# datavizweb/async-rl-tensorflow

Measured on NVIDIA B200. Metric: env_frames_per_sec, higher is better.
Workload: dtype f32

## Files before the change

async-rl-tensorflow_b200/csrc/api.cu:

```cuda
#include <stdarg.h>
#include <stdlib.h>
#include <string.h>

#include "common.cuh"

namespace arl {

static thread_local char g_err[512] = "";

void set_error(const char* fmt, ...) {
  va_list ap;
  va_start(ap, fmt);
  vsnprintf(g_err, sizeof(g_err), fmt, ap);
  va_end(ap);
}

int cuda_fail(cudaError_t e, const char* what) {
  set_error("CUDA error %d (%s) at %s", (int)e, cudaGetErrorString(e), what);
  return ARL_ERR_CUDA;
}

static long long g_launches = 0;
void count_launch() { __atomic_fetch_add(&g_launches, 1, __ATOMIC_RELAXED); }

static int g_num_sms[64] = {0};
int num_sms() {
  int dev = 0;
  if (cudaGetDevice(&dev) != cudaSuccess) dev = 0;
  const int n = g_num_sms[dev & 63];
  return n > 0 ? n : 148;
}

int preprocess_init(int device);
int conv_init();
int heads_init();

}

using namespace arl;

extern "C" const char* arl_last_error(void) { return g_err; }
extern "C" int arl_version(void) { return 100; }
extern "C" int64_t arl_launch_count(int reset) {
  const long long v = __atomic_load_n(&g_launches, __ATOMIC_RELAXED);
  if (reset) __atomic_store_n(&g_launches, 0, __ATOMIC_RELAXED);
  return (int64_t)v;
}

extern "C" int arl_init(int device) {
  int count = 0;
  ARL_CUDA(cudaGetDeviceCount(&count));
  ARL_REQUIRE(device >= 0 && device < count, "arl_init: device %d not in [0,%d)", device, count);
  int prev = 0;
  ARL_CUDA(cudaGetDevice(&prev));
  ARL_CUDA(cudaSetDevice(device));
  cudaDeviceProp prop;
  ARL_CUDA(cudaGetDeviceProperties(&prop, device));
  if (prop.major != 10) {
    set_error("arl_init: device %d is sm_%d%d; this library is built for sm_100a (B200) only",
              device, prop.major, prop.minor);
    cudaSetDevice(prev);
    return ARL_ERR_UNSUPPORTED;
  }
  g_num_sms[device & 63] = prop.multiProcessorCount;
  int rc = preprocess_init(device);
  if (rc == ARL_OK) rc = conv_init();
  if (rc == ARL_OK) rc = heads_init();
  cudaSetDevice(prev);
  return rc;
}

extern "C" int arl_param_layout(int action_size, int64_t* offsets) {
  ARL_REQUIRE(offsets, "arl_param_layout: null pointer");
  ARL_REQUIRE(action_size >= 1 && action_size <= ARL_MAX_ACTIONS,
              "arl_param_layout: action_size %d outside [1,%d]", action_size, ARL_MAX_ACTIONS);
  const ParamLayout L = param_layout(action_size);
  memcpy(offsets, L.off, sizeof(L.off));
  return ARL_OK;
}

extern "C" int64_t arl_backward_workspace_bytes(int action_size) {
  (void)action_size;
  return (int64_t)8 * ARL_A2_ELEMS * ARL_FC * sizeof(float) + (1 << 20);
}

extern "C" int64_t arl_a2_block_rows(int num_envs) {
  if (num_envs <= 16384) return num_envs;
  for (int c = 16384; c >= 2048; c -= 128)
    if (num_envs % c == 0) return c;
  return num_envs;
}

static int forward_step(const float* params, float* prepared, int action_size, const uint8_t* ring,
                        int num_envs, int ring_slots, int first_slot, float* a1, float* a2, float* h,
                        float* logits, float* probs, float* value, int32_t* actions, int64_t env_id_base,
                        int64_t step, const int64_t* step_dev, uint64_t seed, void* stream) {
  const int chunk = (int)arl_a2_block_rows(num_envs);
  for (int off = 0; off < num_envs; off += chunk) {
    const int n = num_envs - off < chunk ? num_envs - off : chunk;
    float* a1c = a1 + (size_t)off * 3200;
    float* a2c = a2 + (size_t)off * ARL_A2_ELEMS;
    float* hc = h + (size_t)off * ARL_FC;
    int rc = arl_conv1_forward(prepared, ring + (size_t)off * ring_slots * kPlane, a1c, n, ring_slots,
                               first_slot, 1, stream);
    if (rc) return rc;
    rc = arl_conv2_forward(prepared, a1c, a2c, n, stream);
    if (rc) return rc;
    rc = arl_fc_heads_forward(params, prepared, action_size, a2c, hc, logits + (size_t)off * action_size,
                              probs + (size_t)off * action_size, value + off,
                              actions ? actions + off : nullptr, env_id_base + off, step, step_dev, seed, n,
                              stream);
    if (rc) return rc;
  }
  return ARL_OK;
}

extern "C" int arl_forward(const float* params, float* prepared, int refresh_prepared, int action_size,
                           const uint8_t* ring, int num_envs, int ring_slots, int first_slot, int steps,
                           float* a1, float* a2, float* h, float* logits, float* probs, float* value,
                           void* stream) {
  const int64_t N = (int64_t)num_envs * steps;
  int rc = ARL_OK;
  if (refresh_prepared) rc = arl_prepare_weights(params, prepared, stream);
  if (rc) return rc;
  if (steps == 1)
    return forward_step(params, prepared, action_size, ring, num_envs, ring_slots, first_slot, a1, a2, h,
                        logits, probs, value, nullptr, 0, 0, nullptr, 0, stream);
  rc = arl_conv1_forward(prepared, ring, a1, num_envs, ring_slots, first_slot, steps, stream);
  if (rc) return rc;
  rc = arl_conv2_forward(prepared, a1, a2, N, stream);
  if (rc) return rc;
  return arl_fc_heads_forward(params, prepared, action_size, a2, h, logits, probs, value, nullptr, 0, 0,
                              nullptr, 0, N, stream);
}

extern "C" int arl_forward_sample(const float* params, float* prepared, int refresh_prepared, int action_size,
                                  const uint8_t* ring, int num_envs, int ring_slots, int first_slot,
                                  float* a1, float* a2, float* h, float* logits, float* probs, float* value,
                                  int32_t* actions, int64_t env_id_base, int64_t step,
                                  const int64_t* step_dev, uint64_t seed, void* stream) {
  ARL_REQUIRE(actions, "arl_forward_sample: null pointer");
  int rc = ARL_OK;
  if (refresh_prepared) rc = arl_prepare_weights(params, prepared, stream);
  if (rc) return rc;
  return forward_step(params, prepared, action_size, ring, num_envs, ring_slots, first_slot, a1, a2, h,
                      logits, probs, value, actions, env_id_base, step, step_dev, seed, stream);
}

extern "C" int arl_backward(const float* params, const float* prepared, int action_size,
                            const uint8_t* ring, int num_envs, int ring_slots, int first_slot,
                            int steps, const float* a1,
                            const float* a2, const float* h, const float* dlogits,
                            const float* dvalue, float* d_h, float* d_a2, float* d_a1, float* grads,
                            void* workspace, float tensor_scale, int allreduce, void* stream) {
  ARL_REQUIRE(tensor_scale > 0.f, "arl_backward: tensor_scale must be > 0");
  const int64_t N = (int64_t)num_envs * steps;
  const float unscale = 1.0f / tensor_scale;
  int rc = arl_heads_backward(params, action_size, h, dlogits, dvalue, d_h, grads, workspace, N,
                              tensor_scale, stream);
  if (rc) return rc;
  rc = arl_fc_backward(prepared, a2, arl_a2_block_rows(num_envs), d_h, d_a2, grads, workspace, N, unscale, stream);
  if (rc) return rc;
  const bool comm = allreduce && arl_comm_size() > 1;
  const ParamLayout L = param_layout(action_size);
  static const bool overlap = [] { const char* e = getenv("ARL_ALLREDUCE_OVERLAP"); return e && e[0] == '1'; }();
  if (comm && !overlap) {
    rc = arl_conv2_backward(prepared, a1, d_a2, d_a1, grads, workspace, N, unscale, stream);
    if (rc) return rc;
    rc = arl_conv1_backward(ring, d_a1, grads, workspace, num_envs, ring_slots, first_slot, steps, unscale, stream);
    if (rc) return rc;
    return arl_allreduce_grads(grads, L.off[ARL_NUM_TENSORS], stream);
  }
  if (comm) {
    rc = arl_allreduce_begin(grads, L.off[T_L4W], L.off[ARL_NUM_TENSORS] - L.off[T_L4W], stream);
    if (rc) return rc;
  }
  rc = arl_conv2_backward(prepared, a1, d_a2, d_a1, grads, workspace, N, unscale, stream);
  if (rc) return rc;
  rc = arl_conv1_backward(ring, d_a1, grads, workspace, num_envs, ring_slots, first_slot, steps,
                          unscale, stream);
  if (rc || !comm) return rc;
  rc = arl_allreduce_begin(grads, 0, L.off[T_L4W], stream);
  if (rc) return rc;
// ... 3 lines not shown
```

async-rl-tensorflow_b200/csrc/convs_tc.cu:

```cuda
#include <stdlib.h>

#include "gemm_tc.cuh"

namespace arl {

int reduce_partials(const float* partials, float* out, int num_partials, int n, cudaStream_t stream);
int reduce_partials_scaled(const float* partials, float* out, int num_partials, int n, float alpha,
                           cudaStream_t stream);

namespace {
using tc::TileCoord;
using tc::kTileM;

__device__ __forceinline__ void load8(const float* p, float (&x)[8]) {
  const float4 x0 = __ldg(reinterpret_cast<const float4*>(p));
  const float4 x1 = __ldg(reinterpret_cast<const float4*>(p) + 1);
  x[0] = x0.x; x[1] = x0.y; x[2] = x0.z; x[3] = x0.w;
  x[4] = x1.x; x[5] = x1.y; x[6] = x1.z; x[7] = x1.w;
}
__device__ __forceinline__ TileCoord row_tile(int item) {
  TileCoord t;
  t.mt = item; t.nt = 0; t.ks = 0; t.k_begin = 0; t.k_end = 0;
  return t;
}
// ... 174 lines not shown
  int num_samples;
};
struct Conv1Fwd : tc::PolicyBase {
  using Args = Conv1FwdArgs;
  static constexpr int GW = 21, GROWS = 441, TROWS = 150;
  static constexpr int PL = (TROWS + 1) * 16;
  static constexpr int EPI_SETS = 2, PROD_WARPS = 8, STAGES = 8, STAGE_BYTES = 4 * PL;
  static constexpr int PLB = 49 * 16, B_IMG = 16 * PLB, SCALE_OFF = B_IMG, BIAS_OFF = B_IMG + 16;
  static constexpr int RES_BYTES = B_IMG + 16 + 64;
  static constexpr int ACC_COLS = 64, OUT_COLS = 16, LO_DELTA = 16, SEG = 16;
  static constexpr bool CUSTOM_EPI = true, ACC_LIMBS3 = true;
  static __device__ __forceinline__ int acc_col(int c) { return c; }
  static __device__ __forceinline__ int num_items(const Args& g) { return (int)((g.rows + 127) / 128); }
  static __device__ __forceinline__ TileCoord coord(const Args&, int item) { return row_tile(item); }
  static __device__ __forceinline__ int num_stages(const Args&, const TileCoord&) { return 1; }
  static __device__ __forceinline__ void load_resident(const Args& g, uint8_t* res, int ptid, int nthr) {
    copy_image<RES_BYTES>(res, g.w_img, ptid, nthr);
  }
  static __device__ __forceinline__ void build_image(const float* params, uint8_t* res, int ptid, int nthr) {
    struct { const float* params; } g{params};
    uint32_t* smax = reinterpret_cast<uint32_t*>(res + SCALE_OFF + 12);
    if (ptid == 0) *smax = 0u;
    asm volatile("bar.sync 1, %0;" ::"r"(nthr) : "memory");
    float m = 0.f;
    for (int i = ptid; i < 4096; i += nthr) m = fmaxf(m, fabsf(g.params[i]));
#pragma unroll
    for (int o = 16; o > 0; o >>= 1) m = fmaxf(m, __shfl_xor_sync(0xffffffffu, m, o));
    if ((ptid & 31) == 0) atomicMax(smax, __float_as_uint(m));
    asm volatile("bar.sync 1, %0;" ::"r"(nthr) : "memory");
    const float s = fmaxf(__uint_as_float(*smax), 1e-30f), inv = 1.0f / s;
    if (ptid == 0) {
      float* sc = reinterpret_cast<float*>(res + SCALE_OFF);
      sc[0] = s * (1.0f / 64.0f); sc[1] = s * (1.0f / 8192.0f); sc[2] = s * (1.0f / 1048576.0f);
    }
    for (int ch = ptid; ch < 16 * 16; ch += nthr) {
      const int co = ch & 15, kc = ch >> 4, tap = kc >> 2, c = kc & 3, a = tap >> 1, b = tap & 1;
      uint32_t l0[4] = {0, 0, 0, 0}, l1[4] = {0, 0, 0, 0}, l2[4] = {0, 0, 0, 0};
#pragma unroll
      for (int e = 0; e < 16; ++e) {
        const int i = e >> 2, j = e & 3;
        const float v = g.params[(((4 * a + i) * 8 + 4 * b + j) * 4 + c) * 16 + co] * inv * 64.0f;
        const float r0 = rintf(v), f1 = (v - r0) * 128.0f, r1 = rintf(f1), r2 = rintf((f1 - r1) * 128.0f);
        l0[e >> 2] |= ((uint32_t)(int)r0 & 0xFFu) << (8 * (e & 3));
        l1[e >> 2] |= ((uint32_t)(int)r1 & 0xFFu) << (8 * (e & 3));
        l2[e >> 2] |= ((uint32_t)(int)r2 & 0xFFu) << (8 * (e & 3));
      }
      uint8_t* d = res + kc * PLB + co * 16;
      *reinterpret_cast<uint4*>(d) = make_uint4(l0[0], l0[1], l0[2], l0[3]);
      *reinterpret_cast<uint4*>(d + 16 * 16) = make_uint4(l1[0], l1[1], l1[2], l1[3]);
      *reinterpret_cast<uint4*>(d + 32 * 16) = make_uint4(l2[0], l2[1], l2[2], l2[3]);
    }
    if (ptid < 16) reinterpret_cast<float*>(res + BIAS_OFF)[ptid] = g.params[4096 + ptid];
  }
  static __device__ __forceinline__ void load_stage(const Args& g, const TileCoord& t, int,
                                                    uint8_t* st, int glane, int gsize, Prod&) {
    const int64_t valid = (int64_t)g.num_samples * GROWS - (int64_t)t.mt * 128;
    if (valid >= TROWS) return;
    for (int c = glane; c < TROWS * 4; c += gsize) {
      const int r = c % TROWS, kc = c / TROWS;
      if (r >= valid) *reinterpret_cast<uint4*>(st + kc * PL + r * 16) = make_uint4(0u, 0u, 0u, 0u);
    }
  }
  static __device__ __forceinline__ bool bulk_stage(const Args& g, const TileCoord& t, int, uint8_t* st,
                                                    int glane, int, uint64_t* full) {
    if (glane >= 8) return false;
    const int sgm = glane >> 2, c = glane & 3;
    const int xr0 = t.mt * 128;
    const int n0 = xr0 / GROWS, q0 = xr0 - n0 * GROWS;
    const int first = min(GROWS - q0, TROWS);
    const int n = n0 + sgm;
    int cnt = sgm == 0 ? first : TROWS - first;
    if (n >= g.num_samples) cnt = 0;
    mbar_expect_tx(full, (uint32_t)cnt * 16u);
    if (cnt > 0) {
      const int tt = n / g.geo.num_envs, b = n - tt * g.geo.num_envs;
      const int slot = (g.geo.first_slot + tt + c) % g.geo.ring_slots;
      const uint8_t* src = g.geo.ring + ((size_t)b * g.geo.ring_slots + slot) * kPlane + (sgm == 0 ? q0 : 0) * 16;
      bulk_g2s(st + c * PL + (sgm == 0 ? 0 : first) * 16, src, (uint32_t)cnt * 16u, full);
    }
    return true;
  }
  static __device__ __forceinline__ void issue(const Args&, const TileCoord&, int, uint32_t st,
                                               uint32_t res, uint32_t d) {
    constexpr uint32_t idesc = tc::make_idesc_i8(48);
    const uint64_t da0 = tc::make_sdesc(st, PL), db0 = tc::make_sdesc(res, PLB);
#pragma unroll
    for (int tap = 0; tap < 4; ++tap) {
#pragma unroll
      for (int k32 = 0; k32 < 2; ++k32) {
        const uint64_t da = tc::sdesc_advance(da0, ((tap >> 1) * GW + (tap & 1)) * 16 + 2 * k32 * PL);
        const uint64_t db = tc::sdesc_advance(db0, (tap * 4 + 2 * k32) * PLB);
        tc::umma_i8(d, da, db, idesc, (tap | k32) != 0 ? 1u : 0u);
      }
    }
  }
  static __device__ __forceinline__ void custom_epilogue(const Args& g, const TileCoord& t,
                                                         const uint8_t* res, uint32_t taddr, int row,
                                                         EpiPre&, EpiState&) {
    const float* sc = reinterpret_cast<const float*>(res + SCALE_OFF);
    float v[16];
    {
      float a[8], b[8];
      tc::tmem_ld8_limbs3(taddr, taddr + 16, taddr + 32, sc[0], sc[1], sc[2], a);
      tc::tmem_ld8_limbs3(taddr + 8, taddr + 24, taddr + 40, sc[0], sc[1], sc[2], b);
#pragma unroll
      for (int e = 0; e < 8; ++e) { v[e] = a[e]; v[8 + e] = b[e]; }
    }
    const int xr = t.mt * 128 + row, n = xr / GROWS;
    const int q = xr - n * GROWS, y = q / GW, x = q - y * GW;
    if (n >= g.num_samples || y >= 20 || x >= 20) return;
    const float2* bias = reinterpret_cast<const float2*>(res + BIAS_OFF);
    uint32_t h[8];
#pragma unroll
    for (int e = 0; e < 8; ++e) {
      const float2 bb = bias[e];
      const float o0 = fmaxf(fmaf(v[2 * e], 1.0f / 255.0f, bb.x), 0.f);
      const float o1 = fmaxf(fmaf(v[2 * e + 1], 1.0f / 255.0f, bb.y), 0.f);
      h[e] = tc::pack_h2(o0, o1);
    }
    uint8_t* d = g.a1s + (size_t)n * kA1sSample + a1s_offset(y, x, 0);
    *reinterpret_cast<uint4*>(d) = make_uint4(h[0], h[1], h[2], h[3]);
    *reinterpret_cast<uint4*>(d + kA1sPlane) = make_uint4(h[4], h[5], h[6], h[7]);
  }
};

struct Conv2FwdArgs {
  const uint8_t* w_img;
  const uint8_t* a1s;
  uint8_t* a2s;
  int64_t rows;
  int num_samples;
  int reverse;
};
struct Conv2Fwd : tc::PolicyBase {
  using Args = Conv2FwdArgs;
  static constexpr int GW = 10, GROWS = 100, TROWS = 140;
  static constexpr int PL = (TROWS + 1) * 16, IMG = 8 * PL;
  static constexpr int EPI_SETS = 2, PROD_WARPS = 6, STAGES = 6, STAGE_BYTES = IMG;
  static constexpr int PLB = 65 * 16, B_IMG = 32 * PLB, BIAS_OFF = B_IMG, RES_BYTES = B_IMG + 128;
  static constexpr int ACC_COLS = 64, OUT_COLS = 32, LO_DELTA = 32, SEG = 32;
  static constexpr bool CUSTOM_EPI = true;
  static __device__ __forceinline__ int acc_col(int c) { return c; }
  static __device__ __forceinline__ int num_items(const Args& g) { return (int)((g.rows + 127) / 128); }
  static __device__ __forceinline__ TileCoord coord(const Args& g, int item) {
    return row_tile(g.reverse ? num_items(g) - 1 - item : item);
  }
  static __device__ __forceinline__ int num_stages(const Args&, const TileCoord&) { return 1; }
  static __device__ __forceinline__ void load_resident(const Args& g, uint8_t* res, int ptid, int nthr) {
    copy_image<RES_BYTES>(res, g.w_img, ptid, nthr);
  }
  static __device__ __forceinline__ void build_image(const float* params, uint8_t* res, int ptid, int nthr) {
    const float* w2 = params + 4112;
    if (ptid < 32) reinterpret_cast<float*>(res + BIAS_OFF)[ptid] = params[4112 + 8192 + ptid];
    for (int ch = ptid; ch < 32 * 32; ch += nthr) {
      const int co = ch & 31, kc = ch >> 5;
      const int tap = kc >> 3, ij = (kc >> 1) & 3, chalf = kc & 1;
      const int kh = 2 * (tap >> 1) + (ij >> 1), kw = 2 * (tap & 1) + (ij & 1);
      float x[8];
#pragma unroll
      for (int e = 0; e < 8; ++e) x[e] = w2[((kh * 4 + kw) * 16 + chalf * 8 + e) * 32 + co];
      tc::store_chunk_split_h(res, res + 32 * 16, kc * PLB + co * 16, x);
    }
  }
  static __device__ __forceinline__ void load_stage(const Args& g, const TileCoord& t, int,
                                                    uint8_t* st, int glane, int gsize, Prod&) {
    a1s_zero_tail<TROWS, PL, 8>(st, t.mt * 128, g.num_samples, glane, gsize);
  }
  static __device__ __forceinline__ bool bulk_stage(const Args& g, const TileCoord& t, int, uint8_t* st,
                                                    int glane, int, uint64_t* full) {
    if (glane >= 8) return false;
    mbar_expect_tx(full, a1s_bulk_bytes<TROWS, false>(t.mt * 128, g.num_samples));
    a1s_bulk_issue<TROWS, PL, false>(st, g.a1s, t.mt * 128, g.num_samples, glane, full);
    return true;
  }
  static __device__ __forceinline__ void issue(const Args&, const TileCoord&, int, uint32_t st,
                                               uint32_t res, uint32_t d) {
    constexpr uint32_t idesc64 = tc::make_idesc_h(64);
    const uint64_t da0 = tc::make_sdesc(st, PL), db0 = tc::make_sdesc(res, PLB);
#pragma unroll
    for (int tap = 0; tap < 4; ++tap) {
      const uint32_t aoff = ((tap >> 1) * GW + (tap & 1)) * 16;
#pragma unroll
      for (int k16 = 0; k16 < 4; ++k16) {
        const uint64_t da = tc::sdesc_advance(da0, aoff + 2 * k16 * PL);
        const uint64_t db = tc::sdesc_advance(db0, (tap * 8 + 2 * k16) * PLB);
        tc::umma_f16(d, da, db, idesc64, (tap | k16) != 0 ? 1u : 0u);
      }
    }
  }
  static __device__ __forceinline__ void custom_epilogue(const Args& g, const TileCoord& t, const uint8_t* res,
                                                         uint32_t taddr, int row, EpiPre&, EpiState&) {
    const int xr = t.mt * 128 + row, n = xr / GROWS;
    const int q = xr - n * GROWS, yp = q / GW, xp = q - yp * GW;
    const bool ok = n < g.num_samples && yp < 9 && xp < 9;
    const float4* bias = reinterpret_cast<const float4*>(res + BIAS_OFF);
    const int64_t plane = (int64_t)g.num_samples * 16, part = 324 * plane;
    uint8_t* d = g.a2s + (int64_t)((yp * 9 + xp) * 4) * plane + (int64_t)n * 16;
#pragma unroll
    for (int c8 = 0; c8 < 4; ++c8) {
      float v[8];
      tc::tmem_ld8_sum(taddr + c8 * 8, taddr + 32 + c8 * 8, v);
      if (!ok) continue;
      const float4 b0 = bias[c8 * 2], b1 = bias[c8 * 2 + 1];
      uint4 h, l;
      tc::split2(fmaxf(v[0] + b0.x, 0.f), fmaxf(v[1] + b0.y, 0.f), h.x, l.x);
      tc::split2(fmaxf(v[2] + b0.z, 0.f), fmaxf(v[3] + b0.w, 0.f), h.y, l.y);
      tc::split2(fmaxf(v[4] + b1.x, 0.f), fmaxf(v[5] + b1.y, 0.f), h.z, l.z);
      tc::split2(fmaxf(v[6] + b1.z, 0.f), fmaxf(v[7] + b1.w, 0.f), h.w, l.w);
      *reinterpret_cast<uint4*>(d + c8 * plane) = h;
      *reinterpret_cast<uint4*>(d + part + c8 * plane) = l;
    }
  }
};

struct Conv2DgradArgs {
  const uint8_t* w_img;
  const uint8_t* a1s;
  const float* dy2;
  uint8_t* dy1s;
  float* bias_partials;
  int64_t rows;
  int num_samples;
};
constexpr int kDy1sRows = 441;
struct Conv2Dgrad : tc::PolicyBase {
  using Args = Conv2DgradArgs;
  static constexpr int GW = 11, GROWS = 121, TROWS = 140;
  static constexpr int PL = 146 * 16, IMG = 4 * PL;
  static constexpr int EPI_SETS = 2, PROD_WARPS = 8, STAGES = 4, STAGE_BYTES = 2 * IMG;
  static constexpr int PLB = 129 * 16, RES_BYTES = 16 * PLB;
  static constexpr int ACC_COLS = 128, OUT_COLS = 64, LO_DELTA = 64, SEG = 32;
  static constexpr bool CUSTOM_EPI = true;
  static __device__ __forceinline__ int acc_col(int c) { return c; }
  static __device__ __forceinline__ int num_items(const Args& g) { return (int)((g.rows + 127) / 128); }
  static __device__ __forceinline__ TileCoord coord(const Args&, int item) { return row_tile(item); }
  static __device__ __forceinline__ int num_stages(const Args&, const TileCoord&) { return 1; }
  static __device__ __forceinline__ void load_resident(const Args& g, uint8_t* res, int ptid, int nthr) {
    copy_image<RES_BYTES>(res, g.w_img, ptid, nthr);
  }
  static __device__ __forceinline__ void build_image(const float* params, uint8_t* res, int ptid, int nthr) {
    const float* w2 = params + 4112;
    for (int ch = ptid; ch < 4 * 16 * 16; ch += nthr) {
      const int c = ch & 15, kc = (ch >> 4) & 15, cls = ch >> 8;
      const int tap = kc >> 2, co8 = kc & 3;
      const int kh = (cls >> 1) + 2 * (tap >> 1), kw = (cls & 1) + 2 * (tap & 1);
      float x[8];
      load8(w2 + ((kh * 4 + kw) * 16 + c) * 32 + co8 * 8, x);
      tc::store_chunk_split(res, res + 64 * 16, kc * PLB + (cls * 16 + c) * 16, x);
    }
  }
  static __device__ __forceinline__ void load_stage(const Args& g, const TileCoord& t, int,
                                                    uint8_t* st, int glane, int gsize, Prod&) {
    float unused[4];
    const int z0 = t.mt * 128;
    stream_pixels<GridZ, 8, TROWS, PL, 7, false, false>(st, st + IMG, g.dy2, z0, z0 + TROWS, g.num_samples,
                                                         glane, gsize, unused);
  }
  static __device__ __forceinline__ void issue(const Args&, const TileCoord&, int, uint32_t st,
                                               uint32_t res, uint32_t d) {
    constexpr uint32_t idesc128 = tc::make_idesc(128), idesc64 = tc::make_idesc(64);
#pragma unroll
    const uint64_t da0 = tc::make_sdesc(st, PL), db0 = tc::make_sdesc(res, PLB);
#pragma unroll
    for (int tap = 0; tap < 4; ++tap) {
      const uint32_t aoff = (12 - 11 * (tap >> 1) - (tap & 1)) * 16;
#pragma unroll
// ... 226 lines not shown
    const int kw = 4 * b + j;
    return g.partials + (size_t)t.ks * 4096 + ((i * 8 + kw) * 4 + cin) * 16;
  }
  static __device__ __forceinline__ int64_t seg_offset(const Args&, const TileCoord&, int a) {
    return a * 4 * 8 * 4 * 16;
  }
  static __device__ __forceinline__ float4 finish(const Args&, float4 v, float4) {
    const float s = 1.0f / 255.0f;
    return make_float4(v.x * s, v.y * s, v.z * s, v.w * s);
  }
};

__global__ void __launch_bounds__(256) build_images_kernel(const float* __restrict__ params, uint8_t* prepared) {
  extern __shared__ __align__(128) uint8_t img[];
  const int tid = threadIdx.x;
  int bytes = 0;
  uint8_t* out = prepared;
  if (blockIdx.x == 0) {
    Conv1Fwd::build_image(params, img, tid, 256);
    bytes = Conv1Fwd::RES_BYTES; out += kPrepW1;
  } else if (blockIdx.x == 1) {
    Conv2Fwd::build_image(params, img, tid, 256);
    bytes = Conv2Fwd::RES_BYTES; out += kPrepW2F;
  } else {
    Conv2Dgrad::build_image(params, img, tid, 256);
    bytes = Conv2Dgrad::RES_BYTES; out += kPrepW2D;
  }
  __syncthreads();
  for (int i = tid; i < bytes / 16; i += 256) reinterpret_cast<uint4*>(out)[i] = reinterpret_cast<const uint4*>(img)[i];
}
static_assert(Conv1Fwd::RES_BYTES <= kPrepW1Bytes && Conv2Fwd::RES_BYTES <= kPrepW2FBytes &&
                  Conv2Dgrad::RES_BYTES <= kPrepW2DBytes, "prepared-weight layout");

bool serpentine() {
  static const bool on = [] { const char* e = getenv("ARL_SERPENTINE"); return !(e && e[0] == '0'); }();
  return on;
}

int split_rows(int64_t rows, int want, int* k_chunk) {
  int64_t per = (rows + want - 1) / want;
  per = (per + 127) / 128 * 128;
  *k_chunk = (int)per;
  return (int)((rows + per - 1) / per);
}

}

int conv_prepare(const float* params, void* prepared, cudaStream_t st) {
  build_images_kernel<<<3, 256, 33536, st>>>(params, (uint8_t*)prepared);
  ARL_LAUNCH_CHECK("build_images_kernel");
  return ARL_OK;
}

}

using namespace arl;

static bool aligned16(const void* p) { return (reinterpret_cast<uintptr_t>(p) & 15) == 0; }

extern "C" int arl_conv1_forward(const float* prepared, const uint8_t* ring, float* a1, int num_envs,
                                 int ring_slots, int first_slot, int steps, void* stream) {
  const float* params = prepared;
  ARL_REQUIRE(params && ring && a1, "arl_conv1_forward: null pointer");
  ARL_REQUIRE(num_envs >= 0 && steps >= 0, "arl_conv1_forward: negative size");
  ARL_REQUIRE(ring_slots >= steps + 3 && first_slot >= 0 && first_slot < ring_slots,
              "arl_conv1_forward: ring_slots %d must be >= steps+3 (%d) and first_slot %d inside it",
              ring_slots, steps + 3, first_slot);
  ARL_REQUIRE(aligned16(params) && aligned16(ring) && aligned16(a1),
              "arl_conv1_forward: pointers must be 16-byte aligned");
  const int64_t N = (int64_t)num_envs * steps;
  if (N == 0) return ARL_OK;
  ARL_REQUIRE(N * 441 < (1LL << 31) - 256, "arl_conv1_forward: too many samples");
  Conv1FwdArgs g{reinterpret_cast<const uint8_t*>(prepared) + kPrepW1, {ring, num_envs, ring_slots, first_slot},
                 reinterpret_cast<uint8_t*>(a1), N * 441, (int)N};
  return tc::launch<Conv1Fwd>(g, (int)((g.rows + 127) / 128), (cudaStream_t)stream);
}

extern "C" int arl_conv2_forward(const float* prepared, const float* a1, float* a2,
                                 int64_t num_samples, void* stream) {
  const float* params = prepared;
  ARL_REQUIRE(params && a1 && a2, "arl_conv2_forward: null pointer");
  ARL_REQUIRE(num_samples >= 0 && num_samples < (1LL << 24), "arl_conv2_forward: bad num_samples");
  ARL_REQUIRE(aligned16(params) && aligned16(a1) && aligned16(a2),
              "arl_conv2_forward: pointers must be 16-byte aligned");
  if (num_samples == 0) return ARL_OK;
  Conv2FwdArgs g{reinterpret_cast<const uint8_t*>(prepared) + kPrepW2F, reinterpret_cast<const uint8_t*>(a1),
                 reinterpret_cast<uint8_t*>(a2), num_samples * 100, (int)num_samples, serpentine() ? 1 : 0};
  return tc::launch<Conv2Fwd>(g, (int)((g.rows + 127) / 128), (cudaStream_t)stream);
}

extern "C" int arl_conv1_backward(const uint8_t* ring, const float* d_a1, float* grads,
                                  void* workspace, int num_envs, int ring_slots, int first_slot,
                                  int steps, float grad_unscale, void* stream) {
  ARL_REQUIRE(ring && d_a1 && grads && workspace, "arl_conv1_backward: null pointer");
  ARL_REQUIRE(num_envs >= 0 && steps >= 0, "arl_conv1_backward: negative size");
  ARL_REQUIRE(ring_slots >= steps + 3 && first_slot >= 0 && first_slot < ring_slots,
              "arl_conv1_backward: ring geometry (slots %d, steps %d, first %d)", ring_slots,
              steps, first_slot);
  ARL_REQUIRE(aligned16(ring) && aligned16(d_a1) && aligned16(grads) && aligned16(workspace),
              "arl_conv1_backward: pointers must be 16-byte aligned");
  const int64_t N = (int64_t)num_envs * steps;
  cudaStream_t st = (cudaStream_t)stream;
  if (N == 0) {
    ARL_CUDA(cudaMemsetAsync(grads, 0, 4096 * sizeof(float), st));
    return ARL_OK;
  }
// ... 54 lines not shown
```

async-rl-tensorflow_b200/src/network.py:

```python
import os
from collections import OrderedDict

import numpy as np
import torch

from .. import _cabi

PARAM_NAMES = ("l1_w", "l1_b", "l2_w", "l2_b", "l4_w", "l4_b", "p_w", "p_b", "q_w", "q_b")
A1_ELEMS, A2_ELEMS, FC, DA1_ELEMS = 6400, 2592, 256, 7056
A1_STORE = 3200
DA1_STORE = 3528


def decode_a1(raw, n=None):
    n = raw.shape[0] if n is None else n
    b = raw.reshape(-1)[:n * A1_STORE].view(torch.float16).reshape(n, 2, 2, 2, 10, 10, 8)
    return b.float().permute(0, 4, 1, 5, 2, 3, 6).reshape(n, 20, 20, 16)


def decode_split(raw, rows, cols):
    b = raw.reshape(-1).view(torch.bfloat16).reshape(2, cols // 8, rows, 8)
    return (b[0].float() + b[1].float()).permute(1, 0, 2).reshape(rows, cols)


def encode_split(x):
    rows, cols = x.shape
    hi = x.float().to(torch.bfloat16)
    lo = (x.float() - hi.float()).to(torch.bfloat16)
    b = torch.stack([hi, lo]).reshape(2, rows, cols // 8, 8).permute(0, 2, 1, 3).contiguous()
    return b.view(torch.float32).reshape(rows, cols)


def decode_da1(raw, n):
    b = raw.reshape(-1)[:n * DA1_STORE].view(torch.float16).reshape(2, n, 21, 21, 8)
    return b.float().permute(1, 2, 3, 0, 4).reshape(n, 21, 21, 16)[:, :20, :20]


def param_shapes(action_size):
    return OrderedDict([
        ("l1_w", (8, 8, 4, 16)), ("l1_b", (16,)), ("l2_w", (4, 4, 16, 32)), ("l2_b", (32,)),
        ("l4_w", (A2_ELEMS, FC)), ("l4_b", (FC,)), ("p_w", (FC, action_size)),
        ("p_b", (action_size,)), ("q_w", (FC, 1)), ("q_b", (1,))])


def initial_weights(action_size, seed=123, stddev=0.02):
    g = torch.Generator().manual_seed(int(seed))
    out = OrderedDict()
    for name, shape in param_shapes(action_size).items():
        if name.endswith("_b"):
            out[name] = torch.zeros(shape)
        elif name in ("l1_w", "l2_w"):
            w = torch.empty(shape)
            torch.nn.init.trunc_normal_(w, 0.0, stddev, -2 * stddev, 2 * stddev, generator=g)
            out[name] = w
        else:
            out[name] = torch.randn(shape, generator=g) * stddev
    return out


class Network(object):
    def __init__(self, sess=None, data_format='NHWC', history_length=4, screen_height=84,
                 screen_width=84, action_size=6, activation_fn='relu', initializer=None,
                 gamma=0.99, beta=0.01, global_network=None, global_optim=None, DQN_type='nips',
                 num_envs=256, t_max=5, device='cuda', seed=123, decay=0.99, epsilon=0.1,
# ... 59 lines not shown

    def set_weights(self, weights):
        for name in PARAM_NAMES:
            self.w[name].copy_(torch.as_tensor(np.asarray(weights[name]), dtype=torch.float32))

    def get_weights(self):
        return OrderedDict((k, v.detach().cpu().numpy().copy()) for k, v in self.w.items())

    def copy_from_global(self):
        if self.global_network is not None and self.global_network is not self:
            self.params.copy_(self.global_network.params)

    def _rows(self, t):
        B = self.num_envs
        return slice(t * B, (t + 1) * B)

    timed = None

    def _timed_call(self, name, *args):
        if self.timed is not None and (name in self.timed or '*' in self.timed):
            e0, e1 = torch.cuda.Event(enable_timing=True), torch.cuda.Event(enable_timing=True)
            e0.record()
            _cabi.call(name, *args)
            e1.record()
            self.events.setdefault(name, []).append((e0, e1))
        else:
            _cabi.call(name, *args)

    def _fc_w_stale(self):
        key = (self.params._version, self._param_writes)
        stale = key != self._fc_w_key
        self._fc_w_key = key
        return stale

    def _forward_into(self, history, l1, l2, l4, logits, probs, value, refresh=None):
        P, st = _cabi.ptr, _cabi.stream_ptr()
        B, A = self.num_envs, self.action_size
        refresh = (1 if self._fc_w_stale() else 0) if refresh is None else int(bool(refresh))
        if self.timed is None:
            _cabi.call("arl_forward", P(self.params), P(self.fc_w), refresh, A, P(history.ring), B,
                       history.ring_slots, history.first_slot(0), 1, P(l1), P(l2), P(l4),
                       P(logits), P(probs), P(value), st)
            return
        if refresh:
            _cabi.call("arl_prepare_weights", P(self.params), P(self.fc_w), st)
        self._timed_layers(history, l1, l2, l4, logits, probs, value, None, 0, 0, None, 0)

    def _timed_layers(self, history, l1, l2, l4, logits, probs, value, actions, env_id_base, step, sd, seed):
        P, st = _cabi.ptr, _cabi.stream_ptr()
        B, A = self.num_envs, self.action_size
        c = _cabi.a2_block_rows(B)
        for o in range(0, B, c):
            r = slice(o, o + c)
            self._timed_call("arl_conv1_forward", P(self.fc_w), P(history.ring[r]), P(l1[r]), c,
                             history.ring_slots, history.first_slot(0), 1, st)
            self._timed_call("arl_conv2_forward", P(self.fc_w), P(l1[r]), P(l2[r]), c, st)
            self._timed_call("arl_fc_heads_forward", P(self.params), P(self.fc_w), A, P(l2[r]), P(l4[r]),
                             P(logits[r]), P(probs[r]), P(value[r]),
                             P(actions[r]) if actions is not None else None, int(env_id_base) + o,
                             int(step), sd, int(seed), c, st)

    def forward(self, history, t, refresh=None):
        r = self._rows(t)
        self._forward_into(history, self.l1[r], self.l2[r], self.l4[r], self.policy_logits[r],
                           self.policy[r], self.value[r], refresh)
        return self.policy_logits[r], self.policy[r], self.value[r]

    def forward_sample(self, history, t, step, seed, env_id_base=0, step_dev=None, refresh=None):
        r = self._rows(t)
        P, st = _cabi.ptr, _cabi.stream_ptr()
        B, A = self.num_envs, self.action_size
        refresh = (1 if self._fc_w_stale() else 0) if refresh is None else int(bool(refresh))
        sd = P(step_dev) if step_dev is not None else None
        if self.timed is None:
            _cabi.call("arl_forward_sample", P(self.params), P(self.fc_w), refresh, A, P(history.ring), B,
                       history.ring_slots, history.first_slot(0), P(self.l1[r]), P(self.l2[r]),
                       P(self.l4[r]), P(self.policy_logits[r]), P(self.policy[r]), P(self.value[r]),
                       P(self.sampled_action[r]), int(env_id_base), int(step), sd, int(seed), st)
            return self.sampled_action[r]
        if refresh:
            _cabi.call("arl_prepare_weights", P(self.params), P(self.fc_w), st)
        self._timed_layers(history, self.l1[r], self.l2[r], self.l4[r], self.policy_logits[r], self.policy[r],
                           self.value[r], self.sampled_action[r], env_id_base, step, sd, seed)
        return self.sampled_action[r]

    def a1(self):
        return decode_a1(self.l1)

    def a2(self):
        B, c = self.num_envs, _cabi.a2_block_rows(self.num_envs)
        return torch.cat([decode_split(self.l2[t * B + o:t * B + o + c], c, A2_ELEMS)
                          for t in range(self.t_max) for o in range(0, B, c)])

    @staticmethod
    def pick_tensor_scale(grad_scale):
        import math
        e = int(round(math.log2(64.0 / max(float(grad_scale), 1e-30))))
        return float(2.0 ** max(-20, min(40, e)))

    def d_h(self):
        N = self.num_envs * self.t_max
        return decode_split(self.d_l4[:N], N, FC) / self.tensor_scale

    def d_a2(self):
        return self.d_l2 / self.tensor_scale

    def d_a1(self):
        return decode_da1(self.d_l1, self.num_envs * self.t_max) / self.tensor_scale

    def d_h_transposed(self):
        N = self.num_envs * self.t_max
        n8 = (N + 7) // 8 * 8
        b = self.d_l4[N:].reshape(-1).view(torch.bfloat16).reshape(2, n8 // 8, FC, 8)
# ... 201 lines not shown
```

Baseline: 10.93 million.

## Fuse conv1 and conv2 forward into one persistent warp-specialized kernel

Adds a persistent kernel that runs conv1 and conv2 forward for groups of four samples. The conv1 epilogue writes its activations both to global memory (kept for backward) and to a shared-memory image that conv2 then reads directly as its UMMA operand, so conv2 no longer reloads a1 from global memory and one launch is removed. Producer, MMA, and two epilogue warp groups are tied together by mbarriers and double-buffered TMEM accumulators, with conv2 tiles interleaved between conv1 tiles. Batches below 4096 samples keep the old two-kernel path. The cost is high code complexity and shared-memory pressure, with one CTA per SM.

```diff
diff --git a/async-rl-tensorflow_b200/csrc/api.cu b/async-rl-tensorflow_b200/csrc/api.cu
--- a/async-rl-tensorflow_b200/csrc/api.cu
+++ b/async-rl-tensorflow_b200/csrc/api.cu
@@ -33,6 +33,8 @@
 
 int preprocess_init(int device);
 int conv_init();
+int convs_forward(const float* prepared, const uint8_t* ring, int num_envs, int ring_slots, int first_slot,
+                  int steps, float* a1, float* a2, cudaStream_t st);
 int heads_init();
 
 }
@@ -101,10 +103,8 @@
     float* a1c = a1 + (size_t)off * 3200;
     float* a2c = a2 + (size_t)off * ARL_A2_ELEMS;
     float* hc = h + (size_t)off * ARL_FC;
-    int rc = arl_conv1_forward(prepared, ring + (size_t)off * ring_slots * kPlane, a1c, n, ring_slots,
-                               first_slot, 1, stream);
-    if (rc) return rc;
-    rc = arl_conv2_forward(prepared, a1c, a2c, n, stream);
+    int rc = convs_forward(prepared, ring + (size_t)off * ring_slots * kPlane, n, ring_slots, first_slot, 1,
+                           a1c, a2c, (cudaStream_t)stream);
     if (rc) return rc;
     rc = arl_fc_heads_forward(params, prepared, action_size, a2c, hc, logits + (size_t)off * action_size,
                               probs + (size_t)off * action_size, value + off,
@@ -126,9 +126,7 @@
   if (steps == 1)
     return forward_step(params, prepared, action_size, ring, num_envs, ring_slots, first_slot, a1, a2, h,
                         logits, probs, value, nullptr, 0, 0, nullptr, 0, stream);
-  rc = arl_conv1_forward(prepared, ring, a1, num_envs, ring_slots, first_slot, steps, stream);
-  if (rc) return rc;
-  rc = arl_conv2_forward(prepared, a1, a2, N, stream);
+  rc = convs_forward(prepared, ring, num_envs, ring_slots, first_slot, steps, a1, a2, (cudaStream_t)stream);
   if (rc) return rc;
   return arl_fc_heads_forward(params, prepared, action_size, a2, h, logits, probs, value, nullptr, 0, 0,
                               nullptr, 0, N, stream);
diff --git a/async-rl-tensorflow_b200/csrc/convs_tc.cu b/async-rl-tensorflow_b200/csrc/convs_tc.cu
--- a/async-rl-tensorflow_b200/csrc/convs_tc.cu
+++ b/async-rl-tensorflow_b200/csrc/convs_tc.cu
@@ -250,33 +250,39 @@
     }
     if (ptid < 16) reinterpret_cast<float*>(res + BIAS_OFF)[ptid] = g.params[4096 + ptid];
   }
-  static __device__ __forceinline__ void load_stage(const Args& g, const TileCoord& t, int,
-                                                    uint8_t* st, int glane, int gsize, Prod&) {
-    const int64_t valid = (int64_t)g.num_samples * GROWS - (int64_t)t.mt * 128;
+  static __device__ __forceinline__ void zero_tail(int num_samples, int xr0, uint8_t* st, int glane, int gsize) {
+    const int64_t valid = (int64_t)num_samples * GROWS - xr0;
     if (valid >= TROWS) return;
     for (int c = glane; c < TROWS * 4; c += gsize) {
       const int r = c % TROWS, kc = c / TROWS;
       if (r >= valid) *reinterpret_cast<uint4*>(st + kc * PL + r * 16) = make_uint4(0u, 0u, 0u, 0u);
     }
   }
-  static __device__ __forceinline__ bool bulk_stage(const Args& g, const TileCoord& t, int, uint8_t* st,
-                                                    int glane, int, uint64_t* full) {
+  static __device__ __forceinline__ void load_stage(const Args& g, const TileCoord& t, int,
+                                                    uint8_t* st, int glane, int gsize, Prod&) {
+    zero_tail(g.num_samples, t.mt * 128, st, glane, gsize);
+  }
+  static __device__ __forceinline__ bool bulk_rows(const RingGeo& geo, int num_samples, int xr0, uint8_t* st,
+                                                   int glane, uint64_t* full) {
     if (glane >= 8) return false;
     const int sgm = glane >> 2, c = glane & 3;
-    const int xr0 = t.mt * 128;
     const int n0 = xr0 / GROWS, q0 = xr0 - n0 * GROWS;
     const int first = min(GROWS - q0, TROWS);
     const int n = n0 + sgm;
     int cnt = sgm == 0 ? first : TROWS - first;
-    if (n >= g.num_samples) cnt = 0;
+    if (n >= num_samples) cnt = 0;
     mbar_expect_tx(full, (uint32_t)cnt * 16u);
     if (cnt > 0) {
-      const int tt = n / g.geo.num_envs, b = n - tt * g.geo.num_envs;
-      const int slot = (g.geo.first_slot + tt + c) % g.geo.ring_slots;
-      const uint8_t* src = g.geo.ring + ((size_t)b * g.geo.ring_slots + slot) * kPlane + (sgm == 0 ? q0 : 0) * 16;
+      const int tt = n / geo.num_envs, b = n - tt * geo.num_envs;
+      const int slot = (geo.first_slot + tt + c) % geo.ring_slots;
+      const uint8_t* src = geo.ring + ((size_t)b * geo.ring_slots + slot) * kPlane + (sgm == 0 ? q0 : 0) * 16;
       bulk_g2s(st + c * PL + (sgm == 0 ? 0 : first) * 16, src, (uint32_t)cnt * 16u, full);
     }
     return true;
+  }
+  static __device__ __forceinline__ bool bulk_stage(const Args& g, const TileCoord& t, int, uint8_t* st,
+                                                    int glane, int, uint64_t* full) {
+    return bulk_rows(g.geo, g.num_samples, t.mt * 128, st, glane, full);
   }
   static __device__ __forceinline__ void issue(const Args&, const TileCoord&, int, uint32_t st,
                                                uint32_t res, uint32_t d) {
@@ -292,9 +298,7 @@
       }
     }
   }
-  static __device__ __forceinline__ void custom_epilogue(const Args& g, const TileCoord& t,
-                                                         const uint8_t* res, uint32_t taddr, int row,
-                                                         EpiPre&, EpiState&) {
+  static __device__ __forceinline__ void epi_values(const uint8_t* res, uint32_t taddr, uint32_t (&h)[8]) {
     const float* sc = reinterpret_cast<const float*>(res + SCALE_OFF);
     float v[16];
     {
@@ -304,11 +308,7 @@
 #pragma unroll
       for (int e = 0; e < 8; ++e) { v[e] = a[e]; v[8 + e] = b[e]; }
     }
-    const int xr = t.mt * 128 + row, n = xr / GROWS;
-    const int q = xr - n * GROWS, y = q / GW, x = q - y * GW;
-    if (n >= g.num_samples || y >= 20 || x >= 20) return;
     const float2* bias = reinterpret_cast<const float2*>(res + BIAS_OFF);
-    uint32_t h[8];
 #pragma unroll
     for (int e = 0; e < 8; ++e) {
       const float2 bb = bias[e];
@@ -316,6 +316,15 @@
       const float o1 = fmaxf(fmaf(v[2 * e + 1], 1.0f / 255.0f, bb.y), 0.f);
       h[e] = tc::pack_h2(o0, o1);
     }
+  }
+  static __device__ __forceinline__ void custom_epilogue(const Args& g, const TileCoord& t,
+                                                         const uint8_t* res, uint32_t taddr, int row,
+                                                         EpiPre&, EpiState&) {
+    uint32_t h[8];
+    epi_values(res, taddr, h);
+    const int xr = t.mt * 128 + row, n = xr / GROWS;
+    const int q = xr - n * GROWS, y = q / GW, x = q - y * GW;
+    if (n >= g.num_samples || y >= 20 || x >= 20) return;
     uint8_t* d = g.a1s + (size_t)n * kA1sSample + a1s_offset(y, x, 0);
     *reinterpret_cast<uint4*>(d) = make_uint4(h[0], h[1], h[2], h[3]);
     *reinterpret_cast<uint4*>(d + kA1sPlane) = make_uint4(h[4], h[5], h[6], h[7]);
@@ -371,29 +380,30 @@
     a1s_bulk_issue<TROWS, PL, false>(st, g.a1s, t.mt * 128, g.num_samples, glane, full);
     return true;
   }
+  template <int APL>
+  static __device__ __forceinline__ void issue_img(uint32_t st, uint32_t res, uint32_t d) {
+    constexpr uint32_t idesc64 = tc::make_idesc_h(64);
+    const uint64_t da0 = tc::make_sdesc(st, APL), db0 = tc::make_sdesc(res, PLB);
+#pragma unroll
+    for (int tap = 0; tap < 4; ++tap) {
+      const uint32_t aoff = ((tap >> 1) * GW + (tap & 1)) * 16;
+#pragma unroll
+      for (int k16 = 0; k16 < 4; ++k16) {
+        const uint64_t da = tc::sdesc_advance(da0, aoff + 2 * k16 * APL);
+        const uint64_t db = tc::sdesc_advance(db0, (tap * 8 + 2 * k16) * PLB);
+        tc::umma_f16(d, da, db, idesc64, (tap | k16) != 0 ? 1u : 0u);
+      }
+    }
+  }
   static __device__ __forceinline__ void issue(const Args&, const TileCoord&, int, uint32_t st,
                                                uint32_t res, uint32_t d) {
-    constexpr uint32_t idesc64 = tc::make_idesc_h(64);
-    const uint64_t da0 = tc::make_sdesc(st, PL), db0 = tc::make_sdesc(res, PLB);
-#pragma unroll
-    for (int tap = 0; tap < 4; ++tap) {
-      const uint32_t aoff = ((tap >> 1) * GW + (tap & 1)) * 16;
-#pragma unroll
-      for (int k16 = 0; k16 < 4; ++k16) {
-        const uint64_t da = tc::sdesc_advance(da0, aoff + 2 * k16 * PL);
-        const uint64_t db = tc::sdesc_advance(db0, (tap * 8 + 2 * k16) * PLB);
-        tc::umma_f16(d, da, db, idesc64, (tap | k16) != 0 ? 1u : 0u);
-      }
-    }
-  }
-  static __device__ __forceinline__ void custom_epilogue(const Args& g, const TileCoord& t, const uint8_t* res,
-                                                         uint32_t taddr, int row, EpiPre&, EpiState&) {
-    const int xr = t.mt * 128 + row, n = xr / GROWS;
-    const int q = xr - n * GROWS, yp = q / GW, xp = q - yp * GW;
-    const bool ok = n < g.num_samples && yp < 9 && xp < 9;
+    issue_img<PL>(st, res, d);
+  }
+  static __device__ __forceinline__ void epi_store(uint8_t* a2s, int num_samples, int n, int yp, int xp, bool ok,
+                                                   const uint8_t* res, uint32_t taddr) {
     const float4* bias = reinterpret_cast<const float4*>(res + BIAS_OFF);
-    const int64_t plane = (int64_t)g.num_samples * 16, part = 324 * plane;
-    uint8_t* d = g.a2s + (int64_t)((yp * 9 + xp) * 4) * plane + (int64_t)n * 16;
+    const int64_t plane = (int64_t)num_samples * 16, part = 324 * plane;
+    uint8_t* d = a2s + (int64_t)((yp * 9 + xp) * 4) * plane + (int64_t)n * 16;
 #pragma unroll
     for (int c8 = 0; c8 < 4; ++c8) {
       float v[8];
@@ -409,7 +419,242 @@
       *reinterpret_cast<uint4*>(d + part + c8 * plane) = l;
     }
   }
-};
+  static __device__ __forceinline__ void custom_epilogue(const Args& g, const TileCoord& t, const uint8_t* res,
+                                                         uint32_t taddr, int row, EpiPre&, EpiState&) {
+    const int xr = t.mt * 128 + row, n = xr / GROWS;
+    const int q = xr - n * GROWS, yp = q / GW, xp = q - yp * GW;
+    epi_store(g.a2s, g.num_samples, n, yp, xp, n < g.num_samples && yp < 9 && xp < 9, res, taddr);
+  }
+};
+
+struct ConvsFwdArgs {
+  const uint8_t* w1_img;
+  const uint8_t* w2_img;
+  RingGeo geo;
+  uint8_t* a1s;
+  uint8_t* a2s;
+  int num_samples, units;
+  int reverse;
+};
+struct ConvsFwd {
+  using C1 = Conv1Fwd;
+  using C2 = Conv2Fwd;
+  static constexpr int G = 4;
+  static constexpr int X2_ROWS = G * 100 + 11;
+  static constexpr int PL2 = (X2_ROWS + 1) * 16, IMG = 8 * PL2;
+  static constexpr int STAGES = 8, EPI1_WARPS = 8, EPI2_WARPS = 8, PROD_WARPS = STAGES;
+  static constexpr int ACC1 = 2, ACC2 = 2;
+  static constexpr uint32_t TMEM_COLS = (ACC1 + ACC2) * 64 <= 256 ? 256 : 512;
+  static constexpr int MMA_WARP = EPI1_WARPS + EPI2_WARPS + PROD_WARPS;
+  static constexpr int THREADS = (MMA_WARP + 1) * 32;
+  static constexpr int RES1_OFF = STAGES * C1::STAGE_BYTES, RES2_OFF = RES1_OFF + C1::RES_BYTES;
+  static constexpr int IMG_OFF = RES2_OFF + C2::RES_BYTES, BAR_OFF = IMG_OFF + 2 * IMG;
+  static constexpr int NBARS = 2 * STAGES + 2 * ACC1 + 2 * ACC2 + 2 * 2;
+  static constexpr int TOTAL = BAR_OFF + NBARS * 8 + 16;
+  static_assert(TOTAL <= 227 * 1024, "shared memory budget (227 KB)");
+  static_assert(RES1_OFF % 16 == 0 && RES2_OFF % 16 == 0 && IMG_OFF % 16 == 0 && BAR_OFF % 8 == 0,
+                "operand images need 16-B alignment");
+
+  struct Unit {
+    int n0, ns, t1, t2;
+  };
+  static __device__ __forceinline__ Unit unit(const ConvsFwdArgs& g, int item) {
+    Unit u;
+    u.n0 = (g.reverse ? g.units - 1 - item : item) * G;
+    u.ns = min(G, g.num_samples - u.n0);
+    u.t1 = (u.ns * 441 + 127) / 128;
+    u.t2 = (u.ns * 100 + 127) / 128;
+    return u;
+  }
+  static __device__ __forceinline__ int t2_start(const Unit& u, int j) {
+    return min(j * 128, max(u.ns * 100 - 128, 0));
+  }
+};
+
+__global__ void __launch_bounds__(ConvsFwd::THREADS, 1) convs_fwd_kernel(ConvsFwdArgs g) {
+  using F = ConvsFwd;
+  using C1 = Conv1Fwd;
+  using C2 = Conv2Fwd;
+  constexpr int STAGES = F::STAGES;
+  extern __shared__ __align__(128) uint8_t smem[];
+  uint8_t* res1 = smem + F::RES1_OFF;
+  uint8_t* res2 = smem + F::RES2_OFF;
+  uint8_t* img = smem + F::IMG_OFF;
+  uint64_t* full = reinterpret_cast<uint64_t*>(smem + F::BAR_OFF);
+  uint64_t* empty = full + STAGES;
+  constexpr int ACC1 = F::ACC1, ACC2 = F::ACC2;
+  uint64_t* t1full = empty + STAGES;
+  uint64_t* t1empty = t1full + ACC1;
+  uint64_t* t2full = t1empty + ACC1;
+  uint64_t* t2empty = t2full + ACC2;
+  uint64_t* a1full = t2empty + ACC2;
+  uint64_t* a1empty = a1full + 2;
+  uint32_t* tmem_slot = reinterpret_cast<uint32_t*>(a1empty + 2);
+  const int tid = threadIdx.x, warp = tid >> 5, lane = tid & 31;
+
+  if (tid == 0) {
+    for (int s = 0; s < STAGES; ++s) {
+      mbar_init(&full[s], 32);
+      mbar_init(&empty[s], 1);
+    }
+    for (int a = 0; a < ACC1; ++a) {
+      mbar_init(&t1full[a], 1);
+      mbar_init(&t1empty[a], 128);
+    }
+    for (int a = 0; a < ACC2; ++a) {
+      mbar_init(&t2full[a], 1);
+      mbar_init(&t2empty[a], 128);
+    }
+    for (int a = 0; a < 2; ++a) {
+      mbar_init(&a1full[a], 32 * F::EPI1_WARPS);
+      mbar_init(&a1empty[a], 1);
+    }
+    fence_mbar_init();
+  }
+  if (warp == F::MMA_WARP) tc::tmem_alloc(tmem_slot, F::TMEM_COLS);
+  if (warp >= F::EPI1_WARPS + F::EPI2_WARPS && warp < F::MMA_WARP) {
+    const int ptid = tid - (F::EPI1_WARPS + F::EPI2_WARPS) * 32;
+    copy_image<C1::RES_BYTES>(res1, g.w1_img, ptid, 32 * F::PROD_WARPS);
+    copy_image<C2::RES_BYTES>(res2, g.w2_img, ptid, 32 * F::PROD_WARPS);
+  }
+  for (int c = tid; c < 2 * 8 * (F::X2_ROWS - F::G * 100); c += F::THREADS) {
+    const int r = F::G * 100 + c % (F::X2_ROWS - F::G * 100), pk = c / (F::X2_ROWS - F::G * 100);
+    *reinterpret_cast<uint4*>(img + pk * F::PL2 + r * 16) = make_uint4(0u, 0u, 0u, 0u);
+  }
+  fence_proxy_async_smem();
+  tc::tc_fence_before();
+  __syncthreads();
+  tc::tc_fence_after();
+  const uint32_t tmem_base = *tmem_slot;
+  asm volatile("griddepcontrol.launch_dependents;" ::: "memory");
+  asm volatile("griddepcontrol.wait;" ::: "memory");
+
+  if (warp >= F::EPI1_WARPS + F::EPI2_WARPS && warp < F::MMA_WARP) {
+    const int pg = warp - (F::EPI1_WARPS + F::EPI2_WARPS);
+    uint8_t* st = smem + pg * C1::STAGE_BYTES;
+    int i = 0;
+    for (int item = blockIdx.x; item < g.units; item += gridDim.x) {
+      const F::Unit u = F::unit(g, item);
+      for (int m = 0; m < u.t1; ++m, ++i) {
+        if (i % STAGES != pg) continue;
+        mbar_wait_backoff<128>(&empty[pg], ((i / STAGES) & 1) ^ 1);
+        const int xr0 = u.n0 * 441 + m * 128;
+        C1::zero_tail(g.num_samples, xr0, st, lane, 32);
+        fence_proxy_async_smem();
+        if (!C1::bulk_rows(g.geo, g.num_samples, xr0, st, lane, &full[pg])) mbar_arrive(&full[pg]);
+      }
+    }
+  } else if (warp == F::MMA_WARP) {
+    const uint32_t res1_addr = smem_u32(res1), res2_addr = smem_u32(res2), img_addr = smem_u32(img);
+    int i = 0, k1 = 0, k2 = 0;
+    F::Unit prev{0, 0, 0, 0};
+    auto conv2_tile = [&](int j, int kk) {
+      const int b = (kk - 1) & 1;
+      if (j == 0) {
+        mbar_wait_sleep(&a1full[b], ((kk - 1) >> 1) & 1);
+        tc::tc_fence_after();
+      }
+      const uint32_t acc = k2 % ACC2;
+      mbar_wait_sleep(&t2empty[acc], ((k2 / ACC2) & 1) ^ 1);
+      tc::tc_fence_after();
+      if (tc::elect_one()) {
+        C2::issue_img<F::PL2>(img_addr + b * F::IMG + F::t2_start(prev, j) * 16, res2_addr,
+                              tmem_base + (ACC1 + acc) * 64);
+        tc::umma_commit(&t2full[acc]);
+        if (j == prev.t2 - 1) tc::umma_commit(&a1empty[b]);
+      }
+      __syncwarp();
+      ++k2;
+    };
+    int kk = 0;
+    for (int item = blockIdx.x;; item += gridDim.x, ++kk) {
+      const bool have = item < g.units;
+      int j2 = 0;
+      const int pt2 = kk > 0 ? prev.t2 : 0;
+      F::Unit u{0, 0, 0, 0};
+      if (have) {
+        u = F::unit(g, item);
+        for (int m = 0; m < u.t1; ++m, ++i, ++k1) {
+          const uint32_t acc = k1 % ACC1;
+          mbar_wait_sleep(&t1empty[acc], ((k1 / ACC1) & 1) ^ 1);
+          tc::tc_fence_after();
+          const int stage = i % STAGES;
+          mbar_wait_sleep(&full[stage], (i / STAGES) & 1);
+          tc::tc_fence_after();
+          if (tc::elect_one()) {
+            C1::issue(C1::Args{}, TileCoord{}, 0, smem_u32(smem + stage * C1::STAGE_BYTES), res1_addr,
+                      tmem_base + acc * 64);
+            tc::umma_commit(&empty[stage]);
+            tc::umma_commit(&t1full[acc]);
+          }
+          __syncwarp();
+          if (m % 3 == 2 && j2 < pt2) conv2_tile(j2++, kk);
+        }
+      }
+      while (j2 < pt2) conv2_tile(j2++, kk);
+      if (!have) break;
+      prev = u;
+    }
+  } else if (warp < F::EPI1_WARPS) {
+    const int quad = warp & 3, set = warp >> 2;
+    int k = 0, kk = 0;
+    for (int item = blockIdx.x; item < g.units; item += gridDim.x, ++kk) {
+      const F::Unit u = F::unit(g, item);
+      const int b = kk & 1;
+      uint8_t* x2 = img + b * F::IMG;
+      mbar_wait_backoff<64>(&a1empty[b], ((kk >> 1) & 1) ^ 1);
+      for (int m = 0; m < u.t1; ++m, ++k) {
+        if ((k & 1) != set) continue;
+        const int acc = k % ACC1;
+        mbar_wait_backoff<64>(&t1full[acc], (k / ACC1) & 1);
+        tc::tc_fence_after();
+        uint32_t h[8];
+        C1::epi_values(res1, tmem_base + ((uint32_t)(quad * 32) << 16) + acc * 64, h);
+        tc::tc_fence_before();
+        mbar_arrive(&t1empty[acc]);
+        const int lr = m * 128 + quad * 32 + lane, s = lr / 441;
+        const int q = lr - s * 441, y = q / 21, x = q - y * 21;
+        if (s < u.ns && y < 20 && x < 20) {
+          const uint4 lo = make_uint4(h[0], h[1], h[2], h[3]), hi = make_uint4(h[4], h[5], h[6], h[7]);
+          uint8_t* d = g.a1s + (size_t)(u.n0 + s) * kA1sSample + a1s_offset(y, x, 0);
+          *reinterpret_cast<uint4*>(d) = lo;
+          *reinterpret_cast<uint4*>(d + kA1sPlane) = hi;
+          uint8_t* e = x2 + (((y & 1) * 2 + (x & 1)) * 2) * F::PL2 + (s * 100 + (y >> 1) * 10 + (x >> 1)) * 16;
+          *reinterpret_cast<uint4*>(e) = lo;
+          *reinterpret_cast<uint4*>(e + F::PL2) = hi;
+        }
+      }
+      fence_proxy_async_smem();
+      mbar_arrive(&a1full[b]);
+    }
+  } else {
+    const int quad = warp & 3, set = (warp - F::EPI1_WARPS) >> 2;
+    int k = 0;
+    for (int item = blockIdx.x; item < g.units; item += gridDim.x) {
+      const F::Unit u = F::unit(g, item);
+      for (int j = 0; j < u.t2; ++j, ++k) {
+        if ((k & 1) != set) continue;
+        const int acc = k % ACC2;
+        mbar_wait_backoff<64>(&t2full[acc], (k / ACC2) & 1);
+        tc::tc_fence_after();
+        const int lr = F::t2_start(u, j) + quad * 32 + lane, s = lr / 100;
+        const int q = lr - s * 100, yp = q / 10, xp = q - yp * 10;
+        const bool ok = lr >= j * 128 && s < u.ns && yp < 9 && xp < 9;
+        C2::epi_store(g.a2s, g.num_samples, u.n0 + s, yp, xp, ok, res2,
+                      tmem_base + ((uint32_t)(quad * 32) << 16) + (ACC1 + acc) * 64);
+        tc::tc_fence_before();
+        mbar_arrive(&t2empty[acc]);
+      }
+    }
+  }
+
+  tc::tc_fence_before();
+  __syncthreads();
+  if (warp == F::MMA_WARP) {
+    tc::tc_fence_after();
+    tc::tmem_dealloc(tmem_base, F::TMEM_COLS);
+  }
+}
 
 struct Conv2DgradArgs {
   const uint8_t* w_img;
@@ -742,6 +987,43 @@
   return ARL_OK;
 }
 
+
+constexpr int64_t kFusedMinSamples = 4096;
+
+int convs_forward(const float* prepared, const uint8_t* ring, int num_envs, int ring_slots, int first_slot,
+                  int steps, float* a1, float* a2, cudaStream_t st) {
+  ARL_REQUIRE(prepared && ring && a1 && a2, "convs_forward: null pointer");
+  ARL_REQUIRE(num_envs >= 0 && steps >= 0, "convs_forward: negative size");
+  ARL_REQUIRE(ring_slots >= steps + 3 && first_slot >= 0 && first_slot < ring_slots,
+              "convs_forward: ring_slots %d must be >= steps+3 (%d) and first_slot %d inside it",
+              ring_slots, steps + 3, first_slot);
+  ARL_REQUIRE(((reinterpret_cast<uintptr_t>(prepared) | reinterpret_cast<uintptr_t>(ring) |
+                reinterpret_cast<uintptr_t>(a1) | reinterpret_cast<uintptr_t>(a2)) & 15) == 0,
+              "convs_forward: pointers must be 16-byte aligned");
+  const int64_t N = (int64_t)num_envs * steps;
+  if (N == 0) return ARL_OK;
+  ARL_REQUIRE(N * 441 < (1LL << 31) - 256, "convs_forward: too many samples");
+  if (N < kFusedMinSamples) {
+    int rc = arl_conv1_forward(prepared, ring, a1, num_envs, ring_slots, first_slot, steps, st);
+    return rc ? rc : arl_conv2_forward(prepared, a1, a2, N, st);
+  }
+  static std::atomic<uint64_t> attr_set{0};
+  int dev = 0;
+  ARL_CUDA(cudaGetDevice(&dev));
+  const uint64_t bit = 1ull << (dev & 63);
+  if (!(attr_set.load(std::memory_order_acquire) & bit)) {
+    ARL_CUDA(cudaFuncSetAttribute(convs_fwd_kernel, cudaFuncAttributeMaxDynamicSharedMemorySize, ConvsFwd::TOTAL));
+    attr_set.fetch_or(bit, std::memory_order_release);
+  }
+  const uint8_t* prep = reinterpret_cast<const uint8_t*>(prepared);
+  ConvsFwdArgs g{prep + kPrepW1, prep + kPrepW2F, {ring, num_envs, ring_slots, first_slot},
+                 reinterpret_cast<uint8_t*>(a1), reinterpret_cast<uint8_t*>(a2), (int)N,
+                 (int)((N + ConvsFwd::G - 1) / ConvsFwd::G), serpentine() ? 1 : 0};
+  ARL_CUDA(launch_pdl(convs_fwd_kernel, dim3(g.units < num_sms() ? g.units : num_sms()), dim3(ConvsFwd::THREADS),
+                      ConvsFwd::TOTAL, st, g));
+  ARL_LAUNCH_CHECK("convs_fwd_kernel");
+  return ARL_OK;
+}
 }
 
 using namespace arl;
diff --git a/async-rl-tensorflow_b200/src/network.py b/async-rl-tensorflow_b200/src/network.py
--- a/async-rl-tensorflow_b200/src/network.py
+++ b/async-rl-tensorflow_b200/src/network.py
@@ -10,6 +10,7 @@
 A1_ELEMS, A2_ELEMS, FC, DA1_ELEMS = 6400, 2592, 256, 7056
 A1_STORE = 3200
 DA1_STORE = 3528
+FUSED_MIN_ENVS = 4096
 
 
 def decode_a1(raw, n=None):
@@ -175,13 +176,23 @@
         c = _cabi.a2_block_rows(B)
         for o in range(0, B, c):
             r = slice(o, o + c)
-            self._timed_call("arl_conv1_forward", P(self.fc_w), P(history.ring[r]), P(l1[r]), c,
-                             history.ring_slots, history.first_slot(0), 1, st)
-            self._timed_call("arl_conv2_forward", P(self.fc_w), P(l1[r]), P(l2[r]), c, st)
-            self._timed_call("arl_fc_heads_forward", P(self.params), P(self.fc_w), A, P(l2[r]), P(l4[r]),
-                             P(logits[r]), P(probs[r]), P(value[r]),
-                             P(actions[r]) if actions is not None else None, int(env_id_base) + o,
-                             int(step), sd, int(seed), c, st)
+            if c < FUSED_MIN_ENVS:
+                self._timed_call("arl_conv1_forward", P(self.fc_w), P(history.ring[r]), P(l1[r]), c,
+                                 history.ring_slots, history.first_slot(0), 1, st)
+                self._timed_call("arl_conv2_forward", P(self.fc_w), P(l1[r]), P(l2[r]), c, st)
+                self._timed_call("arl_fc_heads_forward", P(self.params), P(self.fc_w), A, P(l2[r]), P(l4[r]),
+                                 P(logits[r]), P(probs[r]), P(value[r]),
+                                 P(actions[r]) if actions is not None else None, int(env_id_base) + o,
+                                 int(step), sd, int(seed), c, st)
+            elif actions is None:
+                self._timed_call("arl_forward", P(self.params), P(self.fc_w), 0, A, P(history.ring[r]), c,
+                                 history.ring_slots, history.first_slot(0), 1, P(l1[r]), P(l2[r]), P(l4[r]),
+                                 P(logits[r]), P(probs[r]), P(value[r]), st)
+            else:
+                self._timed_call("arl_forward_sample", P(self.params), P(self.fc_w), 0, A, P(history.ring[r]), c,
+                                 history.ring_slots, history.first_slot(0), P(l1[r]), P(l2[r]), P(l4[r]),
+                                 P(logits[r]), P(probs[r]), P(value[r]), P(actions[r]), int(env_id_base) + o,
+                                 int(step), sd, int(seed), st)
 
     def forward(self, history, t, refresh=None):
         r = self._rows(t)
```

Measured after the change: 11.16 million (median of 6 runs). 2.0% higher.
